# kuleshov-group/caduceus

Hardware: AMD Instinct MI355X
Metric: DNA tokens/sec (whole node), hg38-style MLM pre-train step (higher is better)
Workload: dtype bf16; 1 GPU; Caduceus-PS d_model=256 n_layer=16 seqlen=131072 rcps=true MLM fwd+bwd+allreduce+AdamW, 1 seq/GPU; global_batch=1, accumulate_grad_batches=1, seq_len=131072, parallelism=dp1, params=7725312

## Files before the change

caduceus_amd/csrc/addnorm.hip:

```cpp
#include "cad_common.h"
#include "cad_fp8.h"
#include "cad_rownorm.h"
#include "cad_stream.h"

namespace {

#define AN_KMAX 16
#define AN_WAVES 4

__device__ __forceinline__ float wave_sum(float v) { return cad_row_wave_sum(v); }
__device__ __forceinline__ float wave_max(float v) {
#pragma unroll
    for (int m = 32; m >= 1; m >>= 1) v = fmaxf(v, __shfl_xor(v, m));
    return v;
}
template <typename TY>
__device__ __forceinline__ float stored_value(float o) { return to_f32(from_f32<TY>(o)); }

template <typename TX, typename TY>
__global__ __launch_bounds__(64 * AN_WAVES) void add_norm_fwd_kernel(cad_add_norm_args a) {
    const int lane = threadIdx.x & 63;
    const int wave = threadIdx.x >> 6;
    const int64_t R = a.rows_per_strand;
    const int64_t nrows = R * a.n_strands;
// ... 75 lines not shown
    float dw[AN_KMAX], db[AN_KMAX];
#pragma unroll
    for (int k = 0; k < AN_KMAX; ++k) dw[k] = db[k] = 0.f;
    const int64_t row0 = ((int64_t)blockIdx.x * AN_WAVES + wave) * rows_per_wave;
    for (int i = 0; i < rows_per_wave; ++i) {
        const int64_t row = row0 + i;
        if (row >= nrows) break;
        const int s = row >= R ? 1 : 0;
        const int64_t r = row - (int64_t)s * R;
        const int64_t orow = a.swap_flip ? ((int64_t)(a.n_strands - 1 - s) * R + r) : row;
        const float rstd = a.rstd[row];
        const float mean = (a.is_rms || !a.mean) ? 0.f : a.mean[row];
        float g[AN_KMAX], xh[AN_KMAX];
        float sg = 0.f, sgx = 0.f;
#pragma unroll
        for (int k = 0; k < AN_KMAX; ++k) {
            g[k] = xh[k] = 0.f;
            const int c = lane + 64 * k;
            if (k < kiter && c < D) {
                const int oc = a.swap_flip ? (D - 1 - c) : c;
                const float dyv = to_f32(dy[orow * D + oc]);
                xh[k] = (a.sum_saved[orow * D + oc] - mean) * rstd;
                g[k] = dyv * a.weight[oc];
                sg += g[k];
                sgx += g[k] * xh[k];
                dw[k] += dyv * xh[k];
                db[k] += dyv;
            }
        }
        sgx = wave_sum(sgx) * invD;
        sg = a.is_rms ? 0.f : wave_sum(sg) * invD;
#pragma unroll
        for (int k = 0; k < AN_KMAX; ++k) {
            const int c = lane + 64 * k;
            if (k < kiter && c < D) {
                const int oc = a.swap_flip ? (D - 1 - c) : c;
                float d = rstd * (g[k] - sg - xh[k] * sgx);
                if (a.dres_out) d += a.dres_out[orow * D + oc];
                dx[row * D + c] = from_f32<TX>(d);
                if (a.dres_in) a.dres_in[row * D + c] = d;
            }
        }
    }
    for (int pass = 0; pass < 2; ++pass) {
        if (pass == 1 && !a.dbias) break;
#pragma unroll
        for (int k = 0; k < AN_KMAX; ++k) red[wave][lane + 64 * k] = pass == 0 ? dw[k] : db[k];
        __syncthreads();
        for (int c = threadIdx.x; c < D; c += blockDim.x) {
            float t = 0.f;
            for (int w = 0; w < AN_WAVES; ++w) t += red[w][c];
            const int oc = a.swap_flip ? (D - 1 - c) : c;
            float* slot = pass == 0 ? wslots : bslots;
            if (t != 0.f) {
                if (slot) slot[(int64_t)blockIdx.x * D + oc] = t;
                else atomicAdd(pass == 0 ? &a.dweight[oc] : &a.dbias[oc], t);
            }
        }
        __syncthreads();
    }
}


#define ANV_KMAX 4

template <typename T>
__device__ __forceinline__ void ld4(const T* p, float* o);
template <>
__device__ __forceinline__ void ld4<float>(const float* p, float* o) {
    struct __attribute__((aligned(16))) V { float f[4]; };
    const V t = *(const V*)p;
    o[0] = t.f[0], o[1] = t.f[1], o[2] = t.f[2], o[3] = t.f[3];
}
template <>
__device__ __forceinline__ void ld4<bf16_t>(const bf16_t* p, float* o) {
    struct __attribute__((aligned(8))) V { uint32_t w[2]; };
    const V t = *(const V*)p;
    o[0] = cad_bits2f(t.w[0] << 16), o[1] = cad_bits2f(t.w[0] & 0xffff0000u);
    o[2] = cad_bits2f(t.w[1] << 16), o[3] = cad_bits2f(t.w[1] & 0xffff0000u);
}
template <>
__device__ __forceinline__ void ld4<f16_t>(const f16_t* p, float* o) {
    cad_ld4_16<f16_t>(p, o);
}

template <typename TX, typename TY, int KMAX, bool FP8 = false>
__global__ __launch_bounds__(64 * AN_WAVES) void add_norm_fwd_vec_kernel(cad_add_norm_args a) {
    const int lane = threadIdx.x & 63;
    const int wave = threadIdx.x >> 6;
    const int64_t R = a.rows_per_strand;
    const int64_t nrows = R * a.n_strands;
    const int D = a.D;
    const TX* x = (const TX*)a.x;
    TY* y = (TY*)a.y;
    const float invD = 1.0f / (float)D;
    for (int64_t row = (int64_t)blockIdx.x * AN_WAVES + wave; row < nrows; row += (int64_t)gridDim.x * AN_WAVES) {
        const int s = row >= R ? 1 : 0;
        const int64_t r = row - (int64_t)s * R;
        const int64_t orow = a.swap_flip ? ((int64_t)(a.n_strands - 1 - s) * R + r) : row;
        float v[KMAX][4];
        float s1 = 0.f, s2 = 0.f;
#pragma unroll
        for (int k = 0; k < KMAX; ++k) {
            const int c = (lane + 64 * k) * 4;
            if (c < D) {
                ld4<TX>(x + row * D + c, v[k]);
                if (a.residual_in) {
                    float t[4];
                    ld4<float>(a.residual_in + row * D + c, t);
#pragma unroll
// ... 124 lines not shown
            if (c < D) {
                const int oc = a.swap_flip ? (D - 4 - c) : c;
                float dyv[4], sm[4];
                ld4<TY>(dy + orow * D + oc, dyv);
                ld4<float>(a.sum_saved + orow * D + oc, sm);
#pragma unroll
                for (int q = 0; q < 4; ++q) {
                    xh[k][q] = (sm[q] - mean) * rstd;
                    g[k][q] = dyv[q] * wreg[k][q];
                    sg += g[k][q];
                    sgx += g[k][q] * xh[k][q];
                    dw[k][q] += dyv[q] * xh[k][q];
                    db[k][q] += dyv[q];
                }
            } else {
#pragma unroll
                for (int q = 0; q < 4; ++q) g[k][q] = xh[k][q] = 0.f;
            }
        }
        sgx = wave_sum(sgx) * invD;
        sg = a.is_rms ? 0.f : wave_sum(sg) * invD;
#pragma unroll
        for (int k = 0; k < KMAX; ++k) {
            const int c = (lane + 64 * k) * 4;
            if (c < D) {
                const int oc = a.swap_flip ? (D - 4 - c) : c;
                float dro[4] = {0.f, 0.f, 0.f, 0.f}, d[4];
                if (a.dres_out) ld4<float>(a.dres_out + orow * D + oc, dro);
#pragma unroll
                for (int q = 0; q < 4; ++q) {
                    const int qo = a.swap_flip ? (3 - q) : q;
                    d[q] = rstd * (g[k][qo] - sg - xh[k][qo] * sgx) + dro[qo];
                }
                cad_cvt_store_stream<CAD_STREAM_NORM, TX, 4>(dx + row * D + c, d);
                if (a.dres_in) cad_cvt_store_stream<CAD_STREAM_NORM, float, 4>(a.dres_in + row * D + c, d);
            }
        }
    }
    for (int pass = 0; pass < 2; ++pass) {
        if (pass == 1 && !a.dbias) break;
#pragma unroll
        for (int k = 0; k < KMAX; ++k) {
            const int c = (lane + 64 * k) * 4;
            const int oc = a.swap_flip ? (D - 4 - c) : c;
#pragma unroll
            for (int q = 0; q < 4; ++q)
                if (c < D) red[wave][oc + q] = pass == 0 ? dw[k][q] : db[k][q];
        }
        __syncthreads();
        for (int c = threadIdx.x; c < D; c += blockDim.x) {
            float t = 0.f;
            for (int w = 0; w < AN_WAVES; ++w) t += red[w][c];
            float* slot = pass == 0 ? wslots : bslots;
            if (t != 0.f) {
                if (slot) slot[(int64_t)blockIdx.x * D + c] = t;
                else atomicAdd(pass == 0 ? &a.dweight[c] : &a.dbias[c], t);
            }
        }
        __syncthreads();
    }
}

}

extern "C" int cad_add_norm_fwd(const cad_add_norm_args* a, void* stream) {
    CAD_CHECK_ARG(a && a->x && a->weight && a->y && a->rstd);
    CAD_CHECK_ARG(a->rows_per_strand > 0 && a->D > 0 && (a->n_strands == 1 || a->n_strands == 2));
    CAD_CHECK_ARG(a->is_rms || a->mean);
    if (a->D > 64 * AN_KMAX) return CAD_ERR_UNSUPPORTED;
    CadProfScope prof(4, stream);
    const int64_t nrows = a->rows_per_strand * a->n_strands;
    int64_t nb = (nrows + AN_WAVES - 1) / AN_WAVES;
    if (nb > 8192) nb = 8192;
    dim3 grid((unsigned)nb), block(64 * AN_WAVES);
    const bool vec = (a->D % 4) == 0 && (((uintptr_t)a->x | (uintptr_t)a->residual_in | (uintptr_t)a->weight |
                                          (uintptr_t)a->bias | (uintptr_t)a->y | (uintptr_t)a->residual_out) % 16) == 0;
    if (a->y_fp8) {
        CAD_CHECK_ARG(a->y_scale != nullptr);
        if (!vec || a->D > 512 || ((uintptr_t)a->y_fp8 % 4) != 0) return CAD_ERR_UNSUPPORTED;
    }
#define AN_FWD(TX, TY)                                                                  \
    do {                                                                                \
        if (vec && a->y_fp8 && a->D <= 256)                                             \
            CAD_LAUNCH((add_norm_fwd_vec_kernel<TX, TY, 1, true>), grid, block, 0, stream, *a);  \
        else if (vec && a->y_fp8)                                                       \
            CAD_LAUNCH((add_norm_fwd_vec_kernel<TX, TY, 2, true>), grid, block, 0, stream, *a);  \
        else if (vec && a->D <= 256)                                                    \
            CAD_LAUNCH((add_norm_fwd_vec_kernel<TX, TY, 1>), grid, block, 0, stream, *a);  \
        else if (vec && a->D <= 512)                                                    \
            CAD_LAUNCH((add_norm_fwd_vec_kernel<TX, TY, 2>), grid, block, 0, stream, *a);  \
        else if (vec)                                                                   \
            CAD_LAUNCH((add_norm_fwd_vec_kernel<TX, TY, ANV_KMAX>), grid, block, 0, stream, *a);  \
        else                                                                            \
            CAD_LAUNCH((add_norm_fwd_kernel<TX, TY>), grid, block, 0, stream, *a);      \
    } while (0)
    if (a->x_dtype == CAD_F32 && a->y_dtype == CAD_F32)
        AN_FWD(float, float);
    else if (a->x_dtype == CAD_F32 && a->y_dtype == CAD_BF16)
        AN_FWD(float, bf16_t);
    else if (a->x_dtype == CAD_BF16 && a->y_dtype == CAD_BF16)
        AN_FWD(bf16_t, bf16_t);
    else if (a->x_dtype == CAD_F32 && a->y_dtype == CAD_F16)
        AN_FWD(float, f16_t);
    else if (a->x_dtype == CAD_F16 && a->y_dtype == CAD_F16)
        AN_FWD(f16_t, f16_t);
    else
        return CAD_ERR_UNSUPPORTED;
    return cad_after_launch();
}

// ... 62 lines not shown
```

caduceus_amd/csrc/conv1d.hip:

```cpp
#include "cad_common.h"
#include "cad_stream.h"

namespace {

#define CV_VEC 8
#define CV_WAVES 4
#define CV_THREADS (64 * CV_WAVES)
#define CV_KMAX 4
#define CV_TAPS (2 * CV_KMAX - 1)
#define CV_HALO (CV_KMAX - 1)
#define CV_WAVE_POS (62 * CV_VEC)
#define CV_TILES_BWD 8
#define CV_TILES_FWD 4
#define CV_MAXSETS 2
#define CV_BWD_WAVES 4

struct ConvFwdSets {
    cad_conv1d_args s[CV_MAXSETS];
};
struct ConvBwdSets {
    cad_conv1d_bwd_args s[CV_MAXSETS];
    float* wslots[CV_MAXSETS];
    float* bslots[CV_MAXSETS];
};
// ... 240 lines not shown
        if (it + 1 < CV_TILES_BWD && v + CV_WAVES < nvt) fetch(v + CV_WAVES);
        halo_window(own, xe);
#pragma unroll
        for (int s = 0; s < NSETS; ++s) {
            float g[CV_VEC], dpre[CV_VEC], dpe[CV_VEC + 2 * CV_HALO];
            cvt8<T, VEC>(cg[s], l0_c, L, g);
            auto body = [&](auto dir) {
                constexpr int REV = decltype(dir)::value;
#pragma unroll
                for (int j = 0; j < CV_VEC; ++j) {
                    const float acc = conv4<REV>(W4[s], xe + j, bias[s]);
                    const float sg = cad_sigmoid(acc);
                    dpre[j] = g[j] * sg * (1.f + acc * (1.f - sg));
                }
                halo_window(dpre, dpe);
#pragma unroll
                for (int j = 0; j < CV_VEC; ++j) {
                    o[j] += conv4<!REV>(W4[s], dpe + j, 0.f);
                    const float dm = dpre[j] * useful;
#pragma unroll
                    for (int k = 0; k < CV_KMAX; ++k) part[s][k] += dm * xe[j + (REV ? (CV_TAPS - 1 - k) : k)];
                    part[s][CV_KMAX] += dm;
                }
            };
            const int rev = sb_c < sets.s[s].split ? sets.s[s].rev_lo : sets.s[s].rev_hi;
            if (rev) body(DirTag<1>{}); else body(DirTag<0>{});
        }
        if constexpr (ACC) {
            float add[CV_VEC];
            cvt8<T, VEC>(rdx, l0_c, L, add);
#pragma unroll
            for (int j = 0; j < CV_VEC; ++j) o[j] += add[j];
        }
        if (useful != 0.f) store8v<T, VEC>(dx, l0_c, L, o);
    }
#pragma unroll
    for (int s = 0; s < NSETS; ++s)
#pragma unroll
        for (int m = 0; m <= CV_KMAX; ++m) {
            float v = part[s][m];
#pragma unroll
            for (int sh = 32; sh >= 1; sh >>= 1) v += __shfl_xor(v, sh);
            if (lane == 0) red[wave][s][m] = v;
        }
    __syncthreads();
    const int t = threadIdx.x;
    if (t < NSETS * (CV_KMAX + 1)) {
        const int s = t / (CV_KMAX + 1), k = t % (CV_KMAX + 1);
        const cad_conv1d_bwd_args& a = sets.s[s];
        if (k < CV_KMAX) {
            if (k < a.K) {
                float tot = 0.f;
                for (int wv = 0; wv < CV_WAVES; ++wv) tot += red[wv][s][k + CV_KMAX - a.K];
                if (tot != 0.f) {
                    if (sets.wslots[s]) sets.wslots[s][(int64_t)blockIdx.y * a.E * a.K + e * a.K + k] = tot;
                    else atomicAdd(&a.dw[e * a.K + k], tot);
                }
            }
        } else if (a.dbias) {
            float tot = 0.f;
            for (int wv = 0; wv < CV_WAVES; ++wv) tot += red[wv][s][CV_KMAX];
            if (tot != 0.f) {
                if (sets.bslots[s]) sets.bslots[s][(int64_t)blockIdx.y * a.E + e] = tot;
                else atomicAdd(&a.dbias[e], tot);
            }
        }
    }
}

}

extern "C" int cad_conv1d_fwd_multi(const cad_conv1d_args* sets, int nsets, void* stream) {
    CAD_CHECK_ARG(sets && nsets >= 1 && nsets <= CV_MAXSETS);
    ConvFwdSets ks;
    for (int i = 0; i < nsets; ++i) {
        const cad_conv1d_args* a = &sets[i];
        CAD_CHECK_ARG(a->x && a->w && a->out);
        CAD_CHECK_ARG(a->E > 0 && a->SB > 0 && a->L > 0 && a->K >= 1 && a->K <= CV_KMAX);
        CAD_CHECK_ARG(a->split >= 0 && a->split <= a->SB);
        CAD_CHECK_ARG((int64_t)a->E * a->SB < (1LL << 31));
        CAD_CHECK_ARG(a->x == sets[0].x && a->E == sets[0].E && a->SB == sets[0].SB && a->L == sets[0].L &&
                      a->dtype == sets[0].dtype);
        ks.s[i] = *a;
    }
    for (int i = nsets; i < CV_MAXSETS; ++i) ks.s[i] = sets[0];
    const cad_conv1d_args* a = &sets[0];
    CadProfScope prof(2, stream);
    const int64_t nvt = a->SB * ((a->L + CV_WAVE_POS - 1) / CV_WAVE_POS);
    if (nvt >= (1LL << 31)) return CAD_ERR_UNSUPPORTED;
    const int64_t per_block = (int64_t)CV_WAVES * CV_TILES_FWD;
    dim3 grid((unsigned)a->E, (unsigned)((nvt + per_block - 1) / per_block)), block(CV_THREADS);
    if (grid.y > 65535u) return CAD_ERR_UNSUPPORTED;
    const size_t vb = (a->dtype == CAD_F32 ? 4 : 2) * CV_VEC;
    uintptr_t ptrs = (uintptr_t)a->x;
    for (int i = 0; i < nsets; ++i) ptrs |= (uintptr_t)sets[i].out;
    const bool vec = (a->L % CV_VEC) == 0 && (ptrs % vb) == 0;
#define CV_FWD(T, NS)                                                                   \
    do {                                                                                \
        if (vec)                                                                        \
            CAD_LAUNCH((conv1d_fwd_kernel<T, NS, true>), grid, block, 0, stream, ks);   \
        else                                                                            \
            CAD_LAUNCH((conv1d_fwd_kernel<T, NS, false>), grid, block, 0, stream, ks);  \
    } while (0)
    if (a->dtype == CAD_F32) {
        if (nsets == 1) CV_FWD(float, 1); else CV_FWD(float, 2);
    } else if (a->dtype == CAD_BF16) {
        if (nsets == 1) CV_FWD(bf16_t, 1); else CV_FWD(bf16_t, 2);
    } else if (a->dtype == CAD_F16) {
        if (nsets == 1) CV_FWD(f16_t, 1); else CV_FWD(f16_t, 2);
    } else {
        return CAD_ERR_UNSUPPORTED;
    }
#undef CV_FWD
    return cad_after_launch();
}

extern "C" int cad_conv1d_fwd(const cad_conv1d_args* a, void* stream) { return cad_conv1d_fwd_multi(a, 1, stream); }

// ... 17 lines not shown
        CAD_CHECK_ARG(a->E > 0 && a->SB > 0 && a->L > 0 && a->K >= 1 && a->K <= CV_KMAX);
        CAD_CHECK_ARG(a->split >= 0 && a->split <= a->SB);
        CAD_CHECK_ARG(a->x == sets[0].x && a->dx == sets[0].dx && a->accumulate == sets[0].accumulate &&
                      a->E == sets[0].E && a->SB == sets[0].SB && a->L == sets[0].L && a->dtype == sets[0].dtype);
        ks.s[i] = *a;
    }
    for (int i = nsets; i < CV_MAXSETS; ++i) ks.s[i] = sets[0];
    const cad_conv1d_bwd_args* a = &sets[0];
    CadProfScope prof(3, stream);
    const int64_t nvt = a->SB * ((a->L + CV_WAVE_POS - 1) / CV_WAVE_POS);
    if (nvt >= (1LL << 31)) return CAD_ERR_UNSUPPORTED;
    const int64_t per_block = (int64_t)CV_WAVES * CV_TILES_BWD;
    dim3 grid((unsigned)a->E, (unsigned)((nvt + per_block - 1) / per_block)), block(CV_THREADS);
    if (grid.y > 65535u) return CAD_ERR_UNSUPPORTED;
    const size_t vb = (a->dtype == CAD_F32 ? 4 : 2) * CV_VEC;
    uintptr_t ptrs = (uintptr_t)a->x | (uintptr_t)a->dx;
    for (int i = 0; i < nsets; ++i) ptrs |= (uintptr_t)sets[i].dout;
    const bool vec = (a->L % CV_VEC) == 0 && (ptrs % vb) == 0;
#define CV_BWD(T, NS)                                                                   \
    do {                                                                                \
        if (vec && a->accumulate)                                                              \
            CAD_LAUNCH((conv1d_bwd_kernel<T, NS, true, true>), grid, block, 0, stream, ks);    \
        else if (vec)                                                                          \
            CAD_LAUNCH((conv1d_bwd_kernel<T, NS, true, false>), grid, block, 0, stream, ks);   \
        else if (a->accumulate)                                                                \
            CAD_LAUNCH((conv1d_bwd_kernel<T, NS, false, true>), grid, block, 0, stream, ks);   \
        else                                                                                   \
            CAD_LAUNCH((conv1d_bwd_kernel<T, NS, false, false>), grid, block, 0, stream, ks);  \
    } while (0)
    if (a->dtype == CAD_F32) {
        if (nsets == 1) CV_BWD(float, 1); else CV_BWD(float, 2);
    } else if (a->dtype == CAD_BF16) {
        if (nsets == 1) CV_BWD(bf16_t, 1); else CV_BWD(bf16_t, 2);
    } else if (a->dtype == CAD_F16) {
        if (nsets == 1) CV_BWD(f16_t, 1); else CV_BWD(f16_t, 2);
    } else {
        return CAD_ERR_UNSUPPORTED;
    }
#undef CV_BWD
    return cad_after_launch();
}

extern "C" int cad_conv1d_bwd_multi(const cad_conv1d_bwd_args* sets, int nsets, void* stream) {
    return conv1d_bwd_multi(sets, nsets, nullptr, nullptr, stream);
}

extern "C" int cad_conv1d_bwd_multi_slotted(const cad_conv1d_bwd_args* sets, int nsets, float* const* wslots, float* const* bslots,
                                            void* stream) {
    CAD_CHECK_ARG(sets && nsets >= 1 && nsets <= CV_MAXSETS && wslots && bslots);
    for (int i = 0; i < nsets; ++i) CAD_CHECK_ARG(wslots[i] && (!sets[i].dbias || bslots[i]));
    const int st = conv1d_bwd_multi(sets, nsets, wslots, bslots, stream);
    if (st != 0) return st;
    const int n = cad_conv1d_bwd_slots(&sets[0]);
    for (int i = 0; i < nsets; ++i) {
        int r = cad_reduce_partials(wslots[i], n, (int64_t)sets[i].E * sets[i].K, sets[i].dw, CAD_F32, stream);
        if (r == 0 && sets[i].dbias) r = cad_reduce_partials(bslots[i], n, sets[i].E, sets[i].dbias, CAD_F32, stream);
        if (r != 0) return r;
    }
    return 0;
}

extern "C" int cad_conv1d_bwd(const cad_conv1d_bwd_args* a, void* stream) { return cad_conv1d_bwd_multi(a, 1, stream); }
```

caduceus_amd/csrc/scan_fold.hip:

```cpp
#include "scan_common.h"

namespace {

template <typename T>
__device__ __forceinline__ void ld4p(const T* p, float* o);
template <>
__device__ __forceinline__ void ld4p<float>(const float* p, float* o) {
    struct __attribute__((aligned(16))) V { float f[4]; };
    const V t = *(const V*)p;
    o[0] = t.f[0], o[1] = t.f[1], o[2] = t.f[2], o[3] = t.f[3];
}
template <>
__device__ __forceinline__ void ld4p<bf16_t>(const bf16_t* p, float* o) {
    struct __attribute__((aligned(8))) V { uint32_t w[2]; };
    const V t = *(const V*)p;
    o[0] = cad_bits2f(t.w[0] << 16), o[1] = cad_bits2f(t.w[0] & 0xffff0000u);
    o[2] = cad_bits2f(t.w[1] << 16), o[3] = cad_bits2f(t.w[1] & 0xffff0000u);
}

template <typename T>
__global__ void reduce_partials_kernel(const typename cad_slot_of<T>::type* src, int nparts, int64_t n, T* dst, int vec) {
    typedef typename cad_slot_of<T>::type TS;
    const int64_t stride = (int64_t)gridDim.x * blockDim.x * 4;
    for (int64_t i = ((int64_t)blockIdx.x * blockDim.x + threadIdx.x) * 4; i < n; i += stride) {
        if (vec && i + 4 <= n) {
            float s[4] = {0.f, 0.f, 0.f, 0.f};
            for (int k0 = 0; k0 < nparts; k0 += CAD_FOLD_GROUP) {
                float g[4] = {0.f, 0.f, 0.f, 0.f};
                for (int k = k0; k < nparts && k < k0 + CAD_FOLD_GROUP; ++k) {
                    float x[4];
                    ld4p<TS>(src + (int64_t)k * n + i, x);
                    g[0] += x[0], g[1] += x[1], g[2] += x[2], g[3] += x[3];
                }
                s[0] += g[0], s[1] += g[1], s[2] += g[2], s[3] += g[3];
            }
            cad_cvt_store<T, 4>(dst + i, s);
        } else {
            for (int64_t q = i; q < n && q < i + 4; ++q) {
                float acc = 0.f;
                for (int k0 = 0; k0 < nparts; k0 += CAD_FOLD_GROUP) {
                    float g = 0.f;
                    for (int k = k0; k < nparts && k < k0 + CAD_FOLD_GROUP; ++k) g += to_f32(src[(int64_t)k * n + q]);
                    acc += g;
                }
                dst[q] = from_f32<T>(acc);
            }
        }
    }
}

struct ReduceJobs {
    const void* src[CAD_REDUCE_MAX_JOBS];
    void* dst[CAD_REDUCE_MAX_JOBS];
};
template <typename T>
__global__ void reduce_partials_multi_kernel(ReduceJobs jobs, int nparts, int64_t n) {
    typedef typename cad_slot_of<T>::type TS;
    const TS* src = (const TS*)jobs.src[blockIdx.y];
    T* dst = (T*)jobs.dst[blockIdx.y];
    const int64_t stride = (int64_t)gridDim.x * blockDim.x * 4;
    for (int64_t i = ((int64_t)blockIdx.x * blockDim.x + threadIdx.x) * 4; i < n; i += stride) {
        float s[4] = {0.f, 0.f, 0.f, 0.f};
        for (int k0 = 0; k0 < nparts; k0 += CAD_FOLD_GROUP) {
            float g[4] = {0.f, 0.f, 0.f, 0.f};
            for (int k = k0; k < nparts && k < k0 + CAD_FOLD_GROUP; ++k) {
                float x[4];
                ld4p<TS>(src + (int64_t)k * n + i, x);
                g[0] += x[0], g[1] += x[1], g[2] += x[2], g[3] += x[3];
            }
            s[0] += g[0], s[1] += g[1], s[2] += g[2], s[3] += g[3];
        }
        cad_cvt_store<T, 4>(dst + i, s);
    }
}

#define FOLD_T 256
#define FOLD_CHUNK 512
static_assert(FOLD_CHUNK == SC_STATE_STEP, "the fold walks the scan backward's chunks (scan_common.h)");
struct FoldSets {
    cad_fold_args s[SC_MAXSETS];
};
__global__ __launch_bounds__(64) void fold_gate_kernel(FoldSets sets, int nsets, int want, uint64_t budget_ticks) {
    if (threadIdx.x != 0) return;
    const uint64_t t0 = cad_wall_clock();
    int last = -1;
    uint64_t t_change = t0;
    for (;;) {
        int n = 0;
        for (int i = 0; i < nsets; ++i) {
            const cad_fold_args& a = sets.s[i];
            n += cad_counter_load_agent(a.counters + a.SB * (a.L / FOLD_CHUNK));
        }
        const uint64_t now = cad_wall_clock();
        if (n >= want) return;
        if (n != last) last = n, t_change = now;
        if (n > 0 && now - t_change >= 2000) return;
        if (now - t0 >= budget_ticks) return;
        cad_poll_sleep();
    }
}
// ... 201 lines not shown
    CAD_CHECK_ARG(flag && result && budget_us > 0 && budget_us <= 1000000);
    CAD_LAUNCH(stream_probe_wait_kernel, dim3(1), dim3(64), 0, stream_a, (const int*)flag, result,
               (uint64_t)budget_us * CAD_WALL_CLOCK_TICKS_PER_US);
    CAD_LAUNCH(stream_probe_set_kernel, dim3(1), dim3(64), 0, stream_b, flag);
    return cad_after_launch();
}

extern "C" int cad_fold_stream_supported(int N, int n_partials, int64_t L, int dtype) {
    if (dtype != CAD_BF16 || N < 1 || L < FOLD_CHUNK || L % FOLD_CHUNK != 0) return 0;
    if (n_partials < CAD_FOLD_GROUP || n_partials > 2048 || (n_partials & (n_partials - 1)) != 0) return 0;
    const int elems = 2 * N * FOLD_CHUNK;
    if (elems % n_partials != 0) return 0;
    const int epw = elems / n_partials;
    if (epw < 8 || epw % 8 != 0) return 0;
    if (n_partials % CAD_FOLD_GROUP != 0) return 0;
    const int vps = epw / 8;
    if ((n_partials / CAD_FOLD_GROUP) * vps > FOLD_T) return 0;
    if (FOLD_CHUNK % epw != 0 && epw % FOLD_CHUNK != 0) return 0;
    if ((N * FOLD_CHUNK) % epw != 0) return 0;
    return 1;
}

extern "C" int cad_fold_partials_stream(const cad_fold_args* sets, int nsets, int mode, void* stream) {
    CAD_CHECK_ARG(sets && nsets >= 1 && nsets <= SC_MAXSETS);
    CAD_CHECK_ARG(mode == CAD_FOLD_CONCURRENT || mode == CAD_FOLD_CLEANUP || mode == CAD_FOLD_ALL);
    FoldSets ks;
    for (int i = 0; i < nsets; ++i) {
        const cad_fold_args* a = &sets[i];
        CAD_CHECK_ARG(a->dB_slots && a->dC_slots && a->dB && a->dC && a->SB > 0 && a->SB <= 65535);
        CAD_CHECK_ARG(a->split >= 0 && a->split <= a->SB);
        if (!cad_fold_stream_supported(a->N, a->n_partials, a->L, a->dtype)) return CAD_ERR_UNSUPPORTED;
        CAD_CHECK_ARG((((uintptr_t)a->dB_slots | (uintptr_t)a->dC_slots | (uintptr_t)a->dB | (uintptr_t)a->dC) % 16) == 0);
        if ((int64_t)a->n_partials * a->N * a->SB * a->L * 2 >= ((int64_t)1 << 32)) return CAD_ERR_UNSUPPORTED;
        CAD_CHECK_ARG(mode != CAD_FOLD_CONCURRENT || (a->counters && a->abort_from));
        CAD_CHECK_ARG(mode != CAD_FOLD_CLEANUP || a->abort_from);
        CAD_CHECK_ARG(a->N == sets[0].N && a->n_partials == sets[0].n_partials && a->L == sets[0].L && a->SB == sets[0].SB);
        ks.s[i] = *a;
    }
    for (int i = nsets; i < SC_MAXSETS; ++i) ks.s[i] = sets[0];
    const uint64_t budget = 2000000ull;
    const int64_t items = (int64_t)sets[0].n_partials * sets[0].SB * nsets;
    const int cus = cad_cu_count();
    if (items > (int64_t)cus * FOLD_MAX_ITEMS) return CAD_ERR_UNSUPPORTED;
    dim3 grid((unsigned)(items < cus ? items : cus)), block(FOLD_T);
    if (mode == CAD_FOLD_CONCURRENT)
        CAD_LAUNCH(fold_gate_kernel, dim3(1), dim3(64), 0, stream, ks, nsets, (int)items, budget);
    CAD_LAUNCH(fold_stream_kernel, grid, block, 0, stream, ks, nsets, mode, budget);
    return cad_after_launch();
}

extern "C" int cad_reduce_partials(const void* src, int n_partials, int64_t n, void* dst, int dst_dtype, void* stream) {
    CAD_CHECK_ARG(src && dst && n_partials >= 1 && n > 0);
    const int vec = (n % 4) == 0 && (((uintptr_t)src | (uintptr_t)dst) % 16) == 0;
    int64_t nb = (n / 4 + 255) / 256 + 1;
    if (nb > 16384) nb = 16384;
    dim3 grid((unsigned)nb), block(256);
    if (dst_dtype == CAD_F32)
        CAD_LAUNCH((reduce_partials_kernel<float>), grid, block, 0, stream, (const float*)src, n_partials, n, (float*)dst, vec);
    else if (dst_dtype == CAD_BF16)
        CAD_LAUNCH((reduce_partials_kernel<bf16_t>), grid, block, 0, stream, (const bf16_t*)src, n_partials, n, (bf16_t*)dst, vec);
    else if (dst_dtype == CAD_F16)
        CAD_LAUNCH((reduce_partials_kernel<f16_t>), grid, block, 0, stream, (const bf16_t*)src, n_partials, n, (f16_t*)dst, vec);
    else
        return CAD_ERR_UNSUPPORTED;
    return cad_after_launch();
}

extern "C" int cad_reduce_partials_multi(const cad_reduce_job* jobs, int njobs, int n_partials, int64_t n, int dst_dtype, void* stream) {
    CAD_CHECK_ARG(jobs && njobs >= 1 && njobs <= CAD_REDUCE_MAX_JOBS && n_partials >= 1 && n > 0);
    ReduceJobs kj;
    bool vec = (n % 4) == 0;
    for (int i = 0; i < CAD_REDUCE_MAX_JOBS; ++i) {
        const cad_reduce_job& j = jobs[i < njobs ? i : 0];
        CAD_CHECK_ARG(j.src && j.dst);
        kj.src[i] = j.src, kj.dst[i] = j.dst;
        vec = vec && (((uintptr_t)j.src | (uintptr_t)j.dst) % 16) == 0;
    }
    if (!vec) {
        for (int i = 0; i < njobs; ++i) {
            const int rc = cad_reduce_partials(jobs[i].src, n_partials, n, jobs[i].dst, dst_dtype, stream);
            if (rc != CAD_OK) return rc;
        }
        return CAD_OK;
    }
    int64_t nb = (n / 4 + 255) / 256 + 1;
    if (nb > 16384) nb = 16384;
    dim3 grid((unsigned)nb, (unsigned)njobs), block(256);
    if (dst_dtype == CAD_F32)
        CAD_LAUNCH((reduce_partials_multi_kernel<float>), grid, block, 0, stream, kj, n_partials, n);
    else if (dst_dtype == CAD_BF16)
        CAD_LAUNCH((reduce_partials_multi_kernel<bf16_t>), grid, block, 0, stream, kj, n_partials, n);
    else if (dst_dtype == CAD_F16)
        CAD_LAUNCH((reduce_partials_multi_kernel<f16_t>), grid, block, 0, stream, kj, n_partials, n);
    else
        return CAD_ERR_UNSUPPORTED;
    return cad_after_launch();
}
```

caduceus_amd/mixer.py:

```python
from __future__ import annotations

import ctypes as C
import os
from collections import namedtuple

import torch

from . import _lib as L
from . import ops

SetParams = namedtuple("SetParams", "conv_w conv_b W_x W_dt dt_bias A_log D")
SetSaved = namedtuple("SetSaved", "xc delta A dbc D dt_bias conv_w conv_b w_x w_dt state A_log")
SetWork = namedtuple("SetWork", "du ddelta dA dD dbias dBC npart")
Meta = namedtuple("Meta", "SB Lq split pdtypes conv_w_shapes win_dt wout_dt delta_is_dt k")
StepCache = namedtuple("StepCache", "versions w_in w_out w_x w_dt A w_inT w_outT w_xT w_dtT w_out2 w_in_fp8")
_DIRS = ((0, 1), (1, 0))


def _flatten(records):
    return [t for r in records for t in r]


def _unflatten(cls, flat, n):
    w = len(cls._fields)
    return [cls(*flat[j * w:(j + 1) * w]) for j in range(n)], flat[n * w:]


def _conv_fwd2(x, params, split, dirs):
    E, SB, Lq = x.shape
    n = len(params)
    args = (L.Conv1dArgs * n)()
    outs = []
    for i, (wf, bf) in enumerate(params):
        out = torch.empty_like(x)
        stream = L.stream_and_check(x, wf, bf, out)
        args[i] = L.Conv1dArgs(L.ptr(x), L.ptr(wf), L.ptr(bf), L.ptr(out), SB, Lq, split, E, wf.shape[1], dirs[i][0],
                               dirs[i][1], L.dtype_code(x.dtype))
        outs.append(out)
    L.check(L.get_lib().cad_conv1d_fwd_multi(args, n, stream), "cad_conv1d_fwd_multi")
    return outs


def _zeros_f32(spec, device):
    sizes = [int(torch.Size(s).numel()) for s, _ in spec.values()]
    offs = [0]
    for n in sizes:
        offs.append(offs[-1] + (n + 3) // 4 * 4)
    flat = torch.zeros((offs[-1],), dtype=torch.float32, device=device)
    return {name: flat[o:o + n].view(dt).view(s) for o, n, (name, (s, dt)) in zip(offs, sizes, spec.items())}


def _conv_bwd2(x, params, douts, dx, split, dirs, bufs=None):
    E, SB, Lq = x.shape
    n = len(params)
    args = (L.Conv1dBwdArgs * n)()
    res, slots = [], []
    for i, (wf, bf) in enumerate(params):
        if bufs is not None:
            dw, db = bufs[i]
        else:
            dw = torch.zeros_like(wf)
            db = None if bf is None else torch.zeros_like(bf)
        stream = L.stream_and_check(x, wf, bf, douts[i], dx, dw, db)
        args[i] = L.Conv1dBwdArgs(L.ptr(x), L.ptr(wf), L.ptr(bf), L.ptr(douts[i]), L.ptr(dx), L.ptr(dw), L.ptr(db), SB, Lq,
                                  split, E, wf.shape[1], dirs[i][0], dirs[i][1], L.dtype_code(x.dtype), 0)
        ns = L.get_lib().cad_conv1d_bwd_slots(C.byref(args[i]))
        ws, bs = ops.wgrad_slots(ns, dw.numel(), x.device), (None if db is None else ops.wgrad_slots(ns, E, x.device))
        res.append((dw, db))
        slots.append((ws, bs))
    wptr = (C.c_void_p * n)(*[ws.data_ptr() for ws, _ in slots])
    bptr = (C.c_void_p * n)(*[0 if bs is None else bs.data_ptr() for _, bs in slots])
    L.check(L.get_lib().cad_conv1d_bwd_multi_slotted(args, n, wptr, bptr, stream), "cad_conv1d_bwd_multi_slotted")
    return res


def _kchunks(T: int) -> int:
    n = 64
    while n > 1 and (T % n != 0 or T // n < 1024):
        n //= 2
    return n


def _wgrad_cm_cm(a_cm: torch.Tensor, b_cm: torch.Tensor) -> torch.Tensor:
    M, T = a_cm.shape
    if a_cm.dtype in (torch.float32, torch.float16):
        return ops.mm_f32(a_cm.float(), b_cm.float().t())
    n = _kchunks(T)
    if b_cm.shape[0] <= 16 and n >= 64 and T % 16 == 0:
        n = 16
    if n == 1:
        return ops.mm(a_cm, b_cm.t()).float()
    Kc = T // n
    return torch.sum(ops.bmm(a_cm.view(M, n, Kc).permute(1, 0, 2), b_cm.view(-1, n, Kc).permute(1, 2, 0)), dim=0,
                     dtype=torch.float32)


def _own_wgrad_chunked_ok(X: torch.Tensor, M: int) -> bool:
    K, T = X.shape
    return K > 512 and K % 512 == 0 and ops.proj_wgrad_only_supported(X, M, 512, T)


def _own_wgrad_chunked(X: torch.Tensor, Y: torch.Tensor) -> torch.Tensor:
    K = X.shape[0]
    return torch.cat([ops.proj_wgrad_only(X[h:h + 512], Y) for h in range(0, K, 512)], dim=1)


def _wgrad_cm_tm(a_cm: torch.Tensor, b_tm: torch.Tensor) -> torch.Tensor:
    M, T = a_cm.shape
    if _OWN_GEMM:
        own = ops.wgrad_cm_tm(a_cm, b_tm)
        if own is not None:
            return own
    if a_cm.dtype in (torch.float32, torch.float16):
        return ops.mm_f32(a_cm.float(), b_tm.float())
    n = _kchunks(T)
    if n == 1:
        return ops.mm(a_cm, b_tm).float()
    Kc = T // n
    return torch.sum(ops.bmm(a_cm.view(M, n, Kc).permute(1, 0, 2), b_tm.view(n, Kc, -1)), dim=0, dtype=torch.float32)

# ... 425 lines not shown
```

caduceus_amd/ops.py:

```python
from __future__ import annotations

import ctypes as C
import math
import os
from typing import Optional, Tuple

import torch

from . import _lib as L


def _zeros_like_f32(t, shape=None):
    return torch.zeros(t.shape if shape is None else shape, dtype=torch.float32, device=t.device)


class _Embed(torch.autograd.Function):
    @staticmethod
    def forward(ctx, ids, weight, comp, n_strands, out_dtype):
        ids = ids.contiguous()
        w = weight.contiguous()
        B, Lq = ids.shape
        V, D = w.shape
        out = torch.empty((n_strands, B, Lq, D), dtype=out_dtype, device=w.device)
        stream = L.stream_and_check(ids, w, comp, out)
        a = L.EmbedArgs(L.ptr(ids), L.ptr(comp), L.ptr(w), L.ptr(out), B, Lq, D, V, n_strands, L.dtype_code(w.dtype),
                        L.dtype_code(out_dtype))
        L.check(L.get_lib().cad_embed_fwd(C.byref(a), stream), "cad_embed_fwd")
        ctx.save_for_backward(ids, comp)
        ctx.meta = (V, D, n_strands, w.dtype)
        return out

    @staticmethod
    def backward(ctx, dout):
        ids, comp = ctx.saved_tensors
        V, D, n_strands, wdt = ctx.meta
        dout = dout.contiguous()
        dw = torch.zeros((V, D), dtype=torch.float32, device=dout.device)
        if V * D * 4 > 64 * 1024:
            flat = ids.reshape(-1)
            dw.index_add_(0, flat, dout[0].reshape(-1, D).float())
            if n_strands == 2:
                dw.index_add_(0, comp[flat], dout[1].reshape(-1, D).float())
            return None, dw.to(wdt), None, None, None
        stream = L.stream_and_check(ids, comp, dout, dw)
        B, Lq = ids.shape
        a = L.EmbedBwdArgs(L.ptr(ids), L.ptr(comp), L.ptr(dout), L.ptr(dw), B, Lq, D, V, n_strands,
                           L.dtype_code(dout.dtype))
        slots = wgrad_slots(L.get_lib().cad_embed_bwd_slots(C.byref(a)), V * D, dout.device)
        L.check(L.get_lib().cad_embed_bwd_slotted(C.byref(a), L.ptr(slots), stream), "cad_embed_bwd_slotted")
        return None, dw.to(wdt), None, None, None


def wgrad_slots(n_slots: int, n: int, device) -> torch.Tensor:
    if n_slots < 1:
        raise RuntimeError("caduceus_amd: a backward kernel reported no workgroups")
    return torch.zeros((n_slots, n), dtype=torch.float32, device=device)


def embed(ids: torch.Tensor, weight: torch.Tensor, comp: Optional[torch.Tensor], n_strands: int,
          out_dtype: torch.dtype = torch.float32) -> torch.Tensor:
    if ids.dtype != torch.int64:
        ids = ids.long()
    if n_strands == 2 and comp is None:
        raise AssertionError("Complement map must be provided for RCPS.")
    return _Embed.apply(ids, weight, comp, n_strands, out_dtype)


FP8_ACTIVATIONS = False


class _AddNorm(torch.autograd.Function):
    @staticmethod
    def forward(ctx, x, residual, weight, bias, eps, is_rms, swap_flip, y_dtype, want_fp8=False):
        x = x.contiguous()
        S, D = x.shape[0], x.shape[-1]
        rows = x.numel() // (S * D)
        w = weight.float().contiguous()
        b = None if bias is None else bias.float().contiguous()
        res = None if residual is None else residual.contiguous()
        if res is not None and res.dtype != torch.float32:
            raise TypeError("caduceus_amd keeps the residual stream in fp32")
        y = torch.empty(x.shape, dtype=y_dtype, device=x.device)
        res_out = torch.empty(x.shape, dtype=torch.float32, device=x.device)
        rstd = torch.empty((S * rows,), dtype=torch.float32, device=x.device)
        mean = None if is_rms else torch.empty((S * rows,), dtype=torch.float32, device=x.device)
        yq = torch.empty(x.shape, dtype=torch.uint8, device=x.device) if want_fp8 else None
        ys = torch.empty((S * rows,), dtype=torch.float32, device=x.device) if want_fp8 else None
        stream = L.stream_and_check(x, res, w, b, y, res_out, rstd, mean, yq, ys)
        a = L.AddNormArgs(L.ptr(x), L.ptr(res), L.ptr(w), L.ptr(b), L.ptr(y), L.ptr(res_out), L.ptr(rstd), L.ptr(mean),
                          rows, S, D, float(eps), int(is_rms), int(swap_flip), L.dtype_code(x.dtype),
                          L.dtype_code(y_dtype), L.ptr(yq), L.ptr(ys))
        L.check(L.get_lib().cad_add_norm_fwd(C.byref(a), stream), "cad_add_norm_fwd")
        ctx.save_for_backward(res_out, rstd, mean, w)
        ctx.meta = (rows, S, D, is_rms, swap_flip, x.dtype, y_dtype, residual is not None, bias is not None,
                    weight.dtype)
        if want_fp8:
            ctx.mark_non_differentiable(yq, ys)
            return y, res_out, yq, ys
        return y, res_out

    @staticmethod
    def backward(ctx, dy, dres_out, *_unused):
        res_out, rstd, mean, w = ctx.saved_tensors
        rows, S, D, is_rms, swap_flip, x_dtype, y_dtype, has_res, has_bias, wdt = ctx.meta
        dy = dy.contiguous()
        dres_out = None if dres_out is None else dres_out.contiguous()
        dx = torch.empty(res_out.shape, dtype=x_dtype, device=dy.device)
        dres_in = torch.empty(res_out.shape, dtype=torch.float32, device=dy.device) if has_res else None
        dw = torch.zeros((D,), dtype=torch.float32, device=dy.device)
        db = torch.zeros((D,), dtype=torch.float32, device=dy.device) if has_bias else None
        stream = L.stream_and_check(dy, dres_out, res_out, rstd, mean, w, dx, dres_in, dw, db)
        a = L.AddNormBwdArgs(L.ptr(dy), L.ptr(dres_out), L.ptr(res_out), L.ptr(rstd), L.ptr(mean), L.ptr(w), L.ptr(dx),
                             L.ptr(dres_in), L.ptr(dw), L.ptr(db), rows, S, D, int(is_rms), int(swap_flip),
                             L.dtype_code(x_dtype), L.dtype_code(y_dtype))
        n = L.get_lib().cad_add_norm_bwd_slots(C.byref(a))
        ws, bs = wgrad_slots(n, D, dy.device), (None if db is None else wgrad_slots(n, D, dy.device))
        L.check(L.get_lib().cad_add_norm_bwd_slotted(C.byref(a), L.ptr(ws), L.ptr(bs), stream), "cad_add_norm_bwd_slotted")
        return dx, dres_in, dw.to(wdt), (None if db is None else db.to(wdt)), None, None, None, None, None


def add_norm(x: torch.Tensor, residual: Optional[torch.Tensor], weight: torch.Tensor, bias: Optional[torch.Tensor],
             eps: float, is_rms: bool, swap_flip: bool, y_dtype: torch.dtype, want_fp8: bool = False) -> Tuple[torch.Tensor, torch.Tensor]:
    if swap_flip and x.shape[0] != 2:
        raise ValueError("swap_flip needs two strands")
    D = int(x.shape[-1])
    if want_fp8 and FP8_ACTIVATIONS and y_dtype == torch.bfloat16 and D % 4 == 0 and D <= 512 and _fp8_epilogue_aligned(x, residual) and \
            bool(L.get_lib().cad_proj_fp8_supported(D)):
        y, res, yq, ys = _AddNorm.apply(x, residual, weight, bias, eps, is_rms, swap_flip, y_dtype, True)
        y._cad_fp8 = (yq, ys, y._version, y.data_ptr(), tuple(y.shape))
        return y, res
    return _AddNorm.apply(x, residual, weight, bias, eps, is_rms, swap_flip, y_dtype)


def _fp8_epilogue_aligned(x, residual) -> bool:
    ok = x.is_contiguous() and x.data_ptr() % 16 == 0 and (x.shape[-1] * x.element_size()) % 16 == 0
    if residual is not None:
        ok = ok and residual.data_ptr() % 16 == 0
    return ok


def fp8_operand_of(y: torch.Tensor):
    rec = getattr(y, "_cad_fp8", None)
    if rec is None or not y.is_contiguous():
        return None
    yq, ys, ver, ptr, shape = rec
    if y._version != ver or y.data_ptr() != ptr or tuple(y.shape) != shape:
        return None
    return yq, ys


class _Conv1d(torch.autograd.Function):
    @staticmethod
    def forward(ctx, x, w, bias, split, rev_lo, rev_hi):
        x = x.contiguous()
        E, SB, Lq = x.shape
        wf = w.float().reshape(E, -1).contiguous()
        bf = None if bias is None else bias.float().contiguous()
        out = torch.empty_like(x)
        stream = L.stream_and_check(x, wf, bf, out)
        a = L.Conv1dArgs(L.ptr(x), L.ptr(wf), L.ptr(bf), L.ptr(out), SB, Lq, split, E, wf.shape[1], rev_lo, rev_hi,
                         L.dtype_code(x.dtype))
        L.check(L.get_lib().cad_conv1d_fwd(C.byref(a), stream), "cad_conv1d_fwd")
        ctx.save_for_backward(x, wf, bf)
        ctx.meta = (split, rev_lo, rev_hi, w.shape, w.dtype, bias is not None)
        return out

    @staticmethod
    def backward(ctx, dout):
        x, wf, bf = ctx.saved_tensors
        split, rev_lo, rev_hi, wshape, wdt, has_bias = ctx.meta
        E, SB, Lq = x.shape
        dout = dout.contiguous()
        dx = torch.empty_like(x)
        dw = torch.zeros_like(wf)
        db = torch.zeros((E,), dtype=torch.float32, device=x.device) if has_bias else None
        stream = L.stream_and_check(x, wf, bf, dout, dx, dw, db)
        a = L.Conv1dBwdArgs(L.ptr(x), L.ptr(wf), L.ptr(bf), L.ptr(dout), L.ptr(dx), L.ptr(dw), L.ptr(db), SB, Lq, split,
                            E, wf.shape[1], rev_lo, rev_hi, L.dtype_code(x.dtype), 0)
        n = L.get_lib().cad_conv1d_bwd_slots(C.byref(a))
        ws, bs = wgrad_slots(n, dw.numel(), x.device), (None if db is None else wgrad_slots(n, E, x.device))
        L.check(L.get_lib().cad_conv1d_bwd_multi_slotted(C.byref(a), 1, (C.c_void_p * 1)(ws.data_ptr()),
                                                         (C.c_void_p * 1)(0 if bs is None else bs.data_ptr()), stream),
                "cad_conv1d_bwd_multi_slotted")
        return dx, dw.reshape(wshape).to(wdt), (None if db is None else db.to(wdt)), None, None, None


def causal_conv1d(x: torch.Tensor, w: torch.Tensor, bias: Optional[torch.Tensor], split: int, rev_lo: int,
                  rev_hi: int) -> torch.Tensor:
    return _Conv1d.apply(x, w, bias, int(split), int(rev_lo), int(rev_hi))


_CU_COUNT = {}


def _cu_count() -> int:
    if not torch.cuda.is_available():
        return 256
    dev = torch.cuda.current_device()
    if dev not in _CU_COUNT:
        _CU_COUNT[dev] = int(torch.cuda.get_device_properties(dev).multi_processor_count)
    return _CU_COUNT[dev]


def lsplit_factor(E: int, SB: int, Lq: int, nsets: int) -> int:
    env = os.environ.get("CADUCEUS_AMD_LSPLIT", "")
    chunk = int(L.get_lib().cad_scan_chunk_len())
    if env:
        k = max(1, int(env))
        return k if Lq % (k * chunk) == 0 else 1
    ok = lambda k: Lq % (k * chunk) == 0 and Lq // k >= 8 * chunk
    wgs = ((E + 7) // 8) * SB * nsets
    k = 1
    while wgs * 2 * k <= _cu_count() and ok(2 * k):
        k *= 2
    return k


def compose_segments(P, S, k: int, split: int, rev_lo: int, rev_hi: int, towards_end: bool):
    E, SBk, N = S.shape
    SB = SBk // k
    P4, S4 = P.view(E, SB, k, N), S.view(E, SB, k, N)
    out = torch.zeros_like(S4)
    for rows, rev in ((slice(0, split), rev_lo), (slice(split, SB), rev_hi)):
        if rows.start >= rows.stop:
            continue
        ascending = (rev == 0) != towards_end
        order = list(range(k)) if ascending else list(range(k - 1, -1, -1))
        v = None
        for j, q in enumerate(order):
            if v is not None:
                out[:, rows, q] = v
            if j + 1 < k:
                v = S4[:, rows, q] if v is None else P4[:, rows, q] * v + S4[:, rows, q]
# ... 1048 lines not shown
```

Baseline: 1.053 million tokens/s.

## Skip zero-fill of weight-grad slots, batch conv reductions, add deep partial reducer

Backward kernels now always write every per-block weight/bias gradient slot, so slot buffers and final dw/db can be allocated with empty instead of zeros. This removes several memset launches per layer. The two conv weight-grad reductions are merged into one multi-job reduction launch, and a new shared-memory tree reducer handles many partials over small vectors. The risk is a correctness gap: any slot or destination the kernels fail to write would now hold garbage, for example dw/db on the atomic fallback path, which were allocated with empty.

```diff
diff --git a/caduceus_amd/csrc/addnorm.hip b/caduceus_amd/csrc/addnorm.hip
--- a/caduceus_amd/csrc/addnorm.hip
+++ b/caduceus_amd/csrc/addnorm.hip
@@ -151,10 +151,8 @@
             for (int w = 0; w < AN_WAVES; ++w) t += red[w][c];
             const int oc = a.swap_flip ? (D - 1 - c) : c;
             float* slot = pass == 0 ? wslots : bslots;
-            if (t != 0.f) {
-                if (slot) slot[(int64_t)blockIdx.x * D + oc] = t;
-                else atomicAdd(pass == 0 ? &a.dweight[oc] : &a.dbias[oc], t);
-            }
+            if (slot) slot[(int64_t)blockIdx.x * D + oc] = t != 0.f ? t : 0.f;
+            else if (t != 0.f) atomicAdd(pass == 0 ? &a.dweight[oc] : &a.dbias[oc], t);
         }
         __syncthreads();
     }
@@ -385,10 +383,8 @@
             float t = 0.f;
             for (int w = 0; w < AN_WAVES; ++w) t += red[w][c];
             float* slot = pass == 0 ? wslots : bslots;
-            if (t != 0.f) {
-                if (slot) slot[(int64_t)blockIdx.x * D + c] = t;
-                else atomicAdd(pass == 0 ? &a.dweight[c] : &a.dbias[c], t);
-            }
+            if (slot) slot[(int64_t)blockIdx.x * D + c] = t != 0.f ? t : 0.f;
+            else if (t != 0.f) atomicAdd(pass == 0 ? &a.dweight[c] : &a.dbias[c], t);
         }
         __syncthreads();
     }
diff --git a/caduceus_amd/csrc/conv1d.hip b/caduceus_amd/csrc/conv1d.hip
--- a/caduceus_amd/csrc/conv1d.hip
+++ b/caduceus_amd/csrc/conv1d.hip
@@ -316,18 +316,14 @@
             if (k < a.K) {
                 float tot = 0.f;
                 for (int wv = 0; wv < CV_WAVES; ++wv) tot += red[wv][s][k + CV_KMAX - a.K];
-                if (tot != 0.f) {
-                    if (sets.wslots[s]) sets.wslots[s][(int64_t)blockIdx.y * a.E * a.K + e * a.K + k] = tot;
-                    else atomicAdd(&a.dw[e * a.K + k], tot);
-                }
+                if (sets.wslots[s]) sets.wslots[s][(int64_t)blockIdx.y * a.E * a.K + e * a.K + k] = tot != 0.f ? tot : 0.f;
+                else if (tot != 0.f) atomicAdd(&a.dw[e * a.K + k], tot);
             }
         } else if (a.dbias) {
             float tot = 0.f;
             for (int wv = 0; wv < CV_WAVES; ++wv) tot += red[wv][s][CV_KMAX];
-            if (tot != 0.f) {
-                if (sets.bslots[s]) sets.bslots[s][(int64_t)blockIdx.y * a.E + e] = tot;
-                else atomicAdd(&a.dbias[e], tot);
-            }
+            if (sets.bslots[s]) sets.bslots[s][(int64_t)blockIdx.y * a.E + e] = tot != 0.f ? tot : 0.f;
+            else if (tot != 0.f) atomicAdd(&a.dbias[e], tot);
         }
     }
 }
@@ -451,6 +447,15 @@
     const int st = conv1d_bwd_multi(sets, nsets, wslots, bslots, stream);
     if (st != 0) return st;
     const int n = cad_conv1d_bwd_slots(&sets[0]);
+    if (nsets == 2 && sets[0].K == sets[1].K && !sets[0].dbias == !sets[1].dbias) {
+        const cad_reduce_job wj[2] = {{wslots[0], sets[0].dw}, {wslots[1], sets[1].dw}};
+        int r = cad_reduce_partials_multi(wj, 2, n, (int64_t)sets[0].E * sets[0].K, CAD_F32, stream);
+        if (r == 0 && sets[0].dbias) {
+            const cad_reduce_job bj[2] = {{bslots[0], sets[0].dbias}, {bslots[1], sets[1].dbias}};
+            r = cad_reduce_partials_multi(bj, 2, n, sets[0].E, CAD_F32, stream);
+        }
+        return r;
+    }
     for (int i = 0; i < nsets; ++i) {
         int r = cad_reduce_partials(wslots[i], n, (int64_t)sets[i].E * sets[i].K, sets[i].dw, CAD_F32, stream);
         if (r == 0 && sets[i].dbias) r = cad_reduce_partials(bslots[i], n, sets[i].E, sets[i].dbias, CAD_F32, stream);
diff --git a/caduceus_amd/csrc/scan_fold.hip b/caduceus_amd/csrc/scan_fold.hip
--- a/caduceus_amd/csrc/scan_fold.hip
+++ b/caduceus_amd/csrc/scan_fold.hip
@@ -46,6 +46,44 @@
                 dst[q] = from_f32<T>(acc);
             }
         }
+    }
+}
+
+#define RPD_T 256
+#define RPD_VPB 4
+#define RPD_MAX_GROUPS 512
+#define RPD_MIN_PARTS 64
+#define RPD_MAX_N 65536
+__global__ __launch_bounds__(RPD_T) void reduce_partials_deep_kernel(const float* src, int nparts, int64_t n, float* dst) {
+    struct __attribute__((aligned(16))) V4 { float f[4]; };
+    __shared__ V4 gs[RPD_MAX_GROUPS][RPD_VPB];
+    const int t = threadIdx.x, v = t % RPD_VPB;
+    const int64_t i = ((int64_t)blockIdx.x * RPD_VPB + v) * 4;
+    const int ngroups = (nparts + CAD_FOLD_GROUP - 1) / CAD_FOLD_GROUP;
+    if (i < n) {
+        for (int grp = t / RPD_VPB; grp < ngroups; grp += RPD_T / RPD_VPB) {
+            const int k0 = grp * CAD_FOLD_GROUP;
+            float x[CAD_FOLD_GROUP][4];
+#pragma unroll
+            for (int k = 0; k < CAD_FOLD_GROUP; ++k) {
+                if (k0 + k < nparts) ld4p<float>(src + (int64_t)(k0 + k) * n + i, x[k]);
+                else x[k][0] = x[k][1] = x[k][2] = x[k][3] = 0.f;
+            }
+            V4 g = {{0.f, 0.f, 0.f, 0.f}};
+#pragma unroll
+            for (int k = 0; k < CAD_FOLD_GROUP; ++k)
+                if (k0 + k < nparts) g.f[0] += x[k][0], g.f[1] += x[k][1], g.f[2] += x[k][2], g.f[3] += x[k][3];
+            gs[grp][v] = g;
+        }
+    }
+    __syncthreads();
+    if (t < RPD_VPB && i < n) {
+        float s[4] = {0.f, 0.f, 0.f, 0.f};
+        for (int grp = 0; grp < ngroups; ++grp) {
+            const V4 g = gs[grp][v];
+            s[0] += g.f[0], s[1] += g.f[1], s[2] += g.f[2], s[3] += g.f[3];
+        }
+        cad_cvt_store<float, 4>(dst + i, s);
     }
 }
 
@@ -353,6 +391,12 @@
 extern "C" int cad_reduce_partials(const void* src, int n_partials, int64_t n, void* dst, int dst_dtype, void* stream) {
     CAD_CHECK_ARG(src && dst && n_partials >= 1 && n > 0);
     const int vec = (n % 4) == 0 && (((uintptr_t)src | (uintptr_t)dst) % 16) == 0;
+    if (dst_dtype == CAD_F32 && vec && n <= RPD_MAX_N && n_partials >= RPD_MIN_PARTS &&
+        (n_partials + CAD_FOLD_GROUP - 1) / CAD_FOLD_GROUP <= RPD_MAX_GROUPS) {
+        dim3 grid((unsigned)((n / 4 + RPD_VPB - 1) / RPD_VPB)), block(RPD_T);
+        CAD_LAUNCH(reduce_partials_deep_kernel, grid, block, 0, stream, (const float*)src, n_partials, n, (float*)dst);
+        return cad_after_launch();
+    }
     int64_t nb = (n / 4 + 255) / 256 + 1;
     if (nb > 16384) nb = 16384;
     dim3 grid((unsigned)nb), block(256);
diff --git a/caduceus_amd/mixer.py b/caduceus_amd/mixer.py
--- a/caduceus_amd/mixer.py
+++ b/caduceus_amd/mixer.py
@@ -65,7 +65,7 @@
         args[i] = L.Conv1dBwdArgs(L.ptr(x), L.ptr(wf), L.ptr(bf), L.ptr(douts[i]), L.ptr(dx), L.ptr(dw), L.ptr(db), SB, Lq,
                                   split, E, wf.shape[1], dirs[i][0], dirs[i][1], L.dtype_code(x.dtype), 0)
         ns = L.get_lib().cad_conv1d_bwd_slots(C.byref(args[i]))
-        ws, bs = ops.wgrad_slots(ns, dw.numel(), x.device), (None if db is None else ops.wgrad_slots(ns, E, x.device))
+        ws, bs = ops.wgrad_slots(ns, dw.numel(), x.device, zero=False), (None if db is None else ops.wgrad_slots(ns, E, x.device, zero=False))
         res.append((dw, db))
         slots.append((ws, bs))
     wptr = (C.c_void_p * n)(*[ws.data_ptr() for ws, _ in slots])
diff --git a/caduceus_amd/ops.py b/caduceus_amd/ops.py
--- a/caduceus_amd/ops.py
+++ b/caduceus_amd/ops.py
@@ -51,10 +51,10 @@
         return None, dw.to(wdt), None, None, None
 
 
-def wgrad_slots(n_slots: int, n: int, device) -> torch.Tensor:
+def wgrad_slots(n_slots: int, n: int, device, zero: bool = True) -> torch.Tensor:
     if n_slots < 1:
         raise RuntimeError("caduceus_amd: a backward kernel reported no workgroups")
-    return torch.zeros((n_slots, n), dtype=torch.float32, device=device)
+    return (torch.zeros if zero else torch.empty)((n_slots, n), dtype=torch.float32, device=device)
 
 
 def embed(ids: torch.Tensor, weight: torch.Tensor, comp: Optional[torch.Tensor], n_strands: int,
@@ -107,14 +107,14 @@
         dres_out = None if dres_out is None else dres_out.contiguous()
         dx = torch.empty(res_out.shape, dtype=x_dtype, device=dy.device)
         dres_in = torch.empty(res_out.shape, dtype=torch.float32, device=dy.device) if has_res else None
-        dw = torch.zeros((D,), dtype=torch.float32, device=dy.device)
-        db = torch.zeros((D,), dtype=torch.float32, device=dy.device) if has_bias else None
+        dw = torch.empty((D,), dtype=torch.float32, device=dy.device)
+        db = torch.empty((D,), dtype=torch.float32, device=dy.device) if has_bias else None
         stream = L.stream_and_check(dy, dres_out, res_out, rstd, mean, w, dx, dres_in, dw, db)
         a = L.AddNormBwdArgs(L.ptr(dy), L.ptr(dres_out), L.ptr(res_out), L.ptr(rstd), L.ptr(mean), L.ptr(w), L.ptr(dx),
                              L.ptr(dres_in), L.ptr(dw), L.ptr(db), rows, S, D, int(is_rms), int(swap_flip),
                              L.dtype_code(x_dtype), L.dtype_code(y_dtype))
         n = L.get_lib().cad_add_norm_bwd_slots(C.byref(a))
-        ws, bs = wgrad_slots(n, D, dy.device), (None if db is None else wgrad_slots(n, D, dy.device))
+        ws, bs = wgrad_slots(n, D, dy.device, zero=False), (None if db is None else wgrad_slots(n, D, dy.device, zero=False))
         L.check(L.get_lib().cad_add_norm_bwd_slotted(C.byref(a), L.ptr(ws), L.ptr(bs), stream), "cad_add_norm_bwd_slotted")
         return dx, dres_in, dw.to(wdt), (None if db is None else db.to(wdt)), None, None, None, None, None
 
@@ -172,13 +172,13 @@
         E, SB, Lq = x.shape
         dout = dout.contiguous()
         dx = torch.empty_like(x)
-        dw = torch.zeros_like(wf)
-        db = torch.zeros((E,), dtype=torch.float32, device=x.device) if has_bias else None
+        dw = torch.empty_like(wf)
+        db = torch.empty((E,), dtype=torch.float32, device=x.device) if has_bias else None
         stream = L.stream_and_check(x, wf, bf, dout, dx, dw, db)
         a = L.Conv1dBwdArgs(L.ptr(x), L.ptr(wf), L.ptr(bf), L.ptr(dout), L.ptr(dx), L.ptr(dw), L.ptr(db), SB, Lq, split,
                             E, wf.shape[1], rev_lo, rev_hi, L.dtype_code(x.dtype), 0)
         n = L.get_lib().cad_conv1d_bwd_slots(C.byref(a))
-        ws, bs = wgrad_slots(n, dw.numel(), x.device), (None if db is None else wgrad_slots(n, E, x.device))
+        ws, bs = wgrad_slots(n, dw.numel(), x.device, zero=False), (None if db is None else wgrad_slots(n, E, x.device, zero=False))
         L.check(L.get_lib().cad_conv1d_bwd_multi_slotted(C.byref(a), 1, (C.c_void_p * 1)(ws.data_ptr()),
                                                          (C.c_void_p * 1)(0 if bs is None else bs.data_ptr()), stream),
                 "cad_conv1d_bwd_multi_slotted")
```

Result: faster. 1.093 million tokens/s (median of 6 runs) (+3.8%).
